# hebench/reference-seal-backend

Hardware: AMD Instinct MI355X
Metric: ciphertext-ops/sec (CKKS ct x ct mul+relin+rescale, N=2^15, L=16) (higher is better)
Workload: dtype u64 (exact residues; fp64-FMA engine for primes < 2^47, u64 Harvey engine with the fold reduction for the 60-bit primes)

## Files before the change

### reference-seal-backend_amd/csrc/he355_api.hip

```cpp
#include <hip/hip_runtime.h>

#include <array>
#include <algorithm>
#include <cerrno>
#include <cstdlib>
#include <cstdio>
#include <cstring>
#include <map>
#include <random>
#include <memory>
#include <stdexcept>
#include <string>
#include <vector>

#include "../../include/he355.h"
#include "device_pool.h"
#include "he355_internal.h"
#include "he355_kernels.h"
#include "he_params.h"
#include "ntt_core.h"
#include "client/he_client.h"
#include "client/multiword.h"

namespace he355 {
// ... 630 lines not shown
                const K1Mode mode = product ? K1_MUL : galois ? K1_GALOIS : K1_CT3;
                launch_k1(env, L, mode, nc, off, src.a, src.b, src.ix, src.table, B, src.addend, in_k3 && product, in_k3 && !product,
                          grouped ? &groups : nullptr, in_k3 && galois);
                key_switch_tail(env, L, nc, S, shape, in_k3 && product ? relin_scaled() : src.key, ops, grouped ? &groups : nullptr, off, ro, fork);
                return;
            }
            if (fork) HIPCHECK(hipEventRecord(fork, env.stream));
        });
        HIPCHECK(hipGetLastError());
        return groups.sum_out != nullptr;
    }
    void key_switch_tail(const KernelEnv &env, int L, u64 nc, const Scratch &S, KsShape shape, const u64 *key, const K3Fuse &ops,
                         const KsGroups *groups, u64 g_off, u64 *rescale_out, hipEvent_t fork)
    {
        const KsBuffers &B = S.ks;
        const size_t N = P.N, LN = (size_t)L * N;
        const int SP = (int)P.K - 1;
        const bool lat = shape == KsShape::Latency;
        launch_k2(env, L, nc, B, nullptr, 0, lat ? kLatTargets : 1);
        if (fork) HIPCHECK(hipEventRecord(fork, env.stream));
        if (lat) {
            u64 *part = latency_partials((size_t)std::max(kLatSplit, kLatSplitU64) * nc * 2 * (L + 1) * N, env.stream == stream2_ ? 1 : 0);
            launch_k3(env, L, nc, B, key, K3_ALL, nullptr, kLatSplit, part, kLatSplitU64);
            launch_k3_combine(env, L, nc, B, kLatSplit, part, kLatSplitU64);
            launch_floor_cols(env, SP, L, nc * 2, B.tpr, B.e, 0, 0, nullptr, 0, kLatTargets);
        } else if (shape == KsShape::Unfused) {
            launch_k3(env, L, nc, B, key, K3_ALL, nullptr, 1, nullptr, 0, groups, g_off);
            launch_floor_cols(env, SP, L, nc * 2, B.tpr, B.e);
        } else {
            launch_k3(env, L, nc, B, key, K3_SPECIAL_ONLY, nullptr, 1, nullptr, 0, groups, g_off);
            K3Fuse f = ops;
            f.cols = B.e; f.c01 = B.c01; f.c01_item_stride = B.c01_item_stride; f.cols2 = nullptr; f.out = nullptr;
            if (rescale_out) {
                launch_floor_cols(env, SP, 1, nc * 2, B.tpr, B.e,  L - 1,  L);
                f.tt_lo = L - 1; f.tt_hi = L;
                launch_k3(env, L, nc, B, key, K3_DATA_ONLY, &f);
                launch_rows_inv_select(env, L - 1, nc * 2, B.c01 + (size_t)(L - 1) * N, (u64)LN, S.rlr);
                launch_floor_cols(env, L - 1, L - 1, nc * 2, S.rlr, S.f, 0, L - 1,  B.tpr, SP);
                f.tt_lo = 0; f.tt_hi = L - 1; f.cols2 = S.f; f.out = rescale_out;
                launch_k3(env, L, nc, B, key, K3_DATA_ONLY, &f);
                return;
            }
            launch_floor_cols(env, SP, L, nc * 2, B.tpr, B.e);
            f.tt_lo = 0; f.tt_hi = L;
            launch_k3(env, L, nc, B, key, K3_DATA_ONLY, &f, 1, nullptr, 0, groups, g_off);
            return;
        }
        FloorRowsArgs fr;
        fr.src_prime = SP; fr.n_tgt = L; fr.n_src = 2;
        fr.cols = B.e;
        fr.tsrc = B.t; fr.tsrc_op_stride = 2 * LN; fr.tsrc_poly_stride = LN;
        fr.addend = B.c01; fr.add_op_stride = B.c01_item_stride; fr.add_poly_stride = LN;
        fr.out = B.c01; fr.out_op_stride = B.c01_item_stride; fr.out_poly_stride = LN;
        fr.tail_prime = rescale_out ? L - 1 : -1;
        fr.tail = S.rlr;
        launch_floor_rows(env, nc, fr);
        if (rescale_out) rescale_tail(env, L, 2, nc, S, B.c01, 2 * LN, rescale_out);
    }
    void rescale_tail(const KernelEnv &env, int L, int size, u64 nc, const Scratch &S, const u64 *src, u64 src_op_stride, u64 *out)
    {
        const size_t N = P.N, LN = (size_t)L * N, L1N = (size_t)(L - 1) * N;
        launch_floor_cols(env, L - 1, L - 1, nc * size, S.rlr, S.f, 0, 0, nullptr, 0, latency_shape(env, nc) ? kLatTargets : 1);
        FloorRowsArgs fr;
        fr.src_prime = L - 1; fr.n_tgt = L - 1; fr.n_src = size;
        fr.cols = S.f;
        fr.tsrc = src; fr.tsrc_op_stride = src_op_stride; fr.tsrc_poly_stride = LN;
        fr.addend = nullptr; fr.add_op_stride = 0; fr.add_poly_stride = 0;
        fr.out = out; fr.out_op_stride = (u64)size * L1N; fr.out_poly_stride = L1N;
        fr.tail_prime = -1; fr.tail = nullptr;
        launch_floor_rows(env, nc, fr);
    }
// ... 1570 lines not shown
```

### reference-seal-backend_amd/csrc/he355_kernels.h

```cpp
#pragma once
#include <hip/hip_runtime.h>

#include <cstdlib>
#include <utility>

#include "device_types.h"
#include "behz_core.h"
#include "bfv_level_core.h"
#include "bfv_noise_core.h"

namespace he355 {

struct FloorConst {
    u64 inv, inv_shoup;
    double inv_d, inv_i;
    u64 half_mod;
    u64 src_mod;
};

struct KernelProbe {
    static constexpr int kCap = 2048;
    hipEvent_t start[kCap], stop[kCap];
    int created = 0, used = 0;
    u64 ops = 0;
// ... 13 lines not shown



struct KsBuffers {
    u64 *c01;
    u64 c01_item_stride;
    u64 *c2n;
    u64 *c2r;
    u64 *d;
    u64 *t;
    u64 *tp;
    u64 *tpr;
    u64 *e;
};
struct KsGroups {
    const uint32_t *const *perm = nullptr;
    const u64 *const *key = nullptr;
    const u32 *src_block = nullptr;
    u32 group_size = 0;
    u64 *sum_out = nullptr;
    const u32 *count = nullptr;
};
constexpr u32 kGroupKeepBit = 0x80000000u;
constexpr int kMoveListCap = 64;
enum K1Mode { K1_MUL = 0, K1_CT3 = 1, K1_GALOIS = 2 };
enum K3Part { K3_ALL = 0, K3_SPECIAL_ONLY = 1, K3_DATA_ONLY = 2 };
struct K3Fuse {
    const u64 *cols;
    u64 *c01;
    u64 c01_item_stride;
    int tt_lo, tt_hi;
    const u64 *cols2;
    u64 *out;
    const u64 *ta = nullptr, *tb = nullptr;
    Indexer tix{};
    u64 t_op_offset = 0;
    int c1_mode = 0;
    const u64 *c1_src = nullptr;
    const u64 *gsrc = nullptr;
    const uint32_t *gperm = nullptr;
    u64 gsrc_op_offset = 0;
};
inline bool k3_can_fuse(const KernelEnv &env) { return env.scheme == 2 && env.K >= 2; }
struct FloorRowsArgs {
    int src_prime, n_tgt, n_src;
    const u64 *cols;
    const u64 *tsrc; u64 tsrc_op_stride, tsrc_poly_stride;
    const u64 *addend; u64 add_op_stride, add_poly_stride;
    u64 *out; u64 out_op_stride, out_poly_stride;
    int tail_prime;
    u64 *tail;
};


struct CrtTablesDev {
    int L, words;
    const u64 *Q, *halfQ, *punct, *inv;
    double Qd;
    u64 t;
};

struct EncTablesDev {
    const uint32_t *slot_index;
    const void *W, *Z;
};

// ... 93 lines not shown
```

### reference-seal-backend_amd/csrc/he355_kernels.hip

```cpp
#include <hip/hip_runtime.h>

#include <cstdio>
#include <cstdlib>
#include <stdexcept>
#include <type_traits>

#include "he355_kernels.h"
#include "ntt_core.h"
#include "client/ckks_codec.h"
#include "client/multiword.h"
#include "client/sampler.h"

#if !defined(HE355_KNS) || !defined(HE355_U64_FOLD)
#error "he355_kernels.hip is compiled once per form of the u64 engine: -DHE355_KNS=ks_shoup -DHE355_U64_FOLD=0 and -DHE355_KNS=ks_fold -DHE355_U64_FOLD=1 (Makefile)"
#endif
namespace he355 {
namespace HE355_KNS {
namespace {

#include "kernel_common.inc"

template <class Ar>
__device__ __forceinline__ void rows_fwd_job(const PrimeDev &P, u64 *row, bool in_raw, u32 rowbase, int lane, u64 *lds, bool valid)
{
// ... 952 lines not shown
        if (valid) store_rowC(A.t + (ok * A.L + tt) * N + rowoff, lane, v);
        return;
    }
    const bool last = A.logn1 == 0;
    u64 *dst = tt < A.L ? A.t + (ok * A.L + tt) * N + rowoff : A.tpr + ok * N + rowoff;
    if (P.f64) {
        const ArF64 ar = make_ar(P, (ArF64 *)nullptr);
        double x[kRowE];
#pragma unroll
        for (int r = 0; r < kRowE; ++r) x[r] = ar.from_canon(v[r]);
        wave_rows_inv(ar, P, last, n1 + a_row, lane, lds[wave], x);
#pragma unroll
        for (int r = 0; r < kRowE; ++r) v[r] = last ? ar.to_canon(x[r]) : ar.to_raw(x[r]);
    } else {
        const ArU64 ar = make_ar(P, (ArU64 *)nullptr);
        u64 x[kRowE];
#pragma unroll
        for (int r = 0; r < kRowE; ++r) x[r] = v[r];
        wave_rows_inv(ar, P, last, n1 + a_row, lane, lds[wave], x);
#pragma unroll
        for (int r = 0; r < kRowE; ++r) v[r] = last ? ar.to_canon(x[r]) : ar.to_raw(x[r]);
    }
    if (valid) store_rowA(dst, lane, v);
}

struct FloorColsArgs {
    const u64 *src;
    u64 *dst;
    int src_prime, n_tgt, K;
    const FloorConst *fc;
    int tgt_first, dst_ntgt;
    const u64 *src2;
    int src2_prime;
    u64 f64_mask;
    int tsplit;
};

template <int LOGN1>
__device__ __forceinline__ void floor_source_column(const PrimeDev &Ps, const u64 *src, int col, u64 c[1 << LOGN1])
{
    constexpr int N1 = 1 << LOGN1;
    if (LOGN1 == 0) {
        c[0] = src[col];
    } else if (Ps.f64) {
        const ArF64 ar = make_ar(Ps, (ArF64 *)nullptr);
        double x[N1];
#pragma unroll
        for (int a = 0; a < N1; ++a) x[a] = ar.from_raw(src[(a << kRowLog) + col]);
        col_inv<ArF64, LOGN1>(ar, x, ctw(Ps.inv), Ps.inv_w0_scaled);
#pragma unroll
        for (int a = 0; a < N1; ++a) c[a] = ar.to_canon(x[a]);
    } else {
        const ArU64 ar = make_ar(Ps, (ArU64 *)nullptr);
        u64 x[N1];
#pragma unroll
        for (int a = 0; a < N1; ++a) x[a] = src[(a << kRowLog) + col];
        col_inv<ArU64, LOGN1>(ar, x, ctw(Ps.inv), Ps.inv_w0_scaled);
#pragma unroll
        for (int a = 0; a < N1; ++a) c[a] = ar.to_canon(x[a]);
    }
    const u64 qs = Ps.q, half = qs >> 1;
#pragma unroll
    for (int a = 0; a < N1; ++a) c[a] = addmod(c[a], half, qs);
}

struct FcnConsts {
    double half1, half2;
    double inv2, inv2_i;
    double pow32, qd, qinv;
    double recentre;
};

template <int LOGN1, bool MERGE, bool WIDE1>
__device__ __forceinline__ void fcn_targets_f64(const FloorColsArgs &A, const PrimeDev *primes, u64 poly, int col, u64 mask,
                                                const typename std::conditional<WIDE1, u64, double>::type (&c)[1 << LOGN1],
                                                const u64 *park , bool wide2, const FcnConsts *ctab)
{
    constexpr int N1 = 1 << LOGN1;
    constexpr u64 N = (u64)N1 << kRowLog;
    constexpr int LA = LOGN1 < 4 ? LOGN1 : 4;
    if (!mask) return;
    const u32 off8 = (u32)col << 3;
// ... 60 lines not shown
        store_word_rows<N1>(poly_rsrc(A.dst + (poly * A.dst_ntgt + t) * N, (u32)N1 * kSlotBytes), off8, v);
        if (!m) break;
        t = tn; wa = wa_n; k = kn;
    }
}

template <int LOGN1, bool MERGE>
__global__ void __launch_bounds__(kBlock, 2) k_floor_colsn(FloorColsArgs A, const PrimeDev *primes)
{
    constexpr int N1 = 1 << LOGN1;
    constexpr u64 N = (u64)N1 << kRowLog;
    const u64 poly = blockIdx.x >> 2;
    const int col = ((blockIdx.x & 3) << 8) | threadIdx.x;
    __shared__ u64 park[MERGE ? N1 : 1][MERGE ? kBlock : 1];
    __shared__ FcnConsts ctab[kMaxPrimes];
    const PrimeDev &Ps = primes[A.src_prime];
    const u64 qs = Ps.q, qs2 = MERGE ? primes[A.src2_prime].q : 0;
    if ((int)threadIdx.x >= A.tgt_first && (int)threadIdx.x < A.tgt_first + A.n_tgt) {
        const int i = threadIdx.x;
        const PrimeDev &Pi = primes[i];
        FcnConsts k;
        k.half1 = (double)A.fc[A.src_prime * A.K + i].half_mod;
        k.half2 = 0; k.inv2 = 0; k.inv2_i = 0;
        int flags = qs > 2 * Pi.q ? 1 : 0;
        if (MERGE) {
            const FloorConst f2 = A.fc[A.src2_prime * A.K + i];
            k.half2 = (double)f2.half_mod; k.inv2 = f2.inv_d; k.inv2_i = f2.inv_i;
            flags |= qs2 > 2 * Pi.q ? 2 : 0;
        }
        k.pow32 = Pi.pow32; k.qd = Pi.qd; k.qinv = Pi.qinv; k.recentre = (double)flags;
        ctab[i] = k;
    }
    u64 c[N1];
    floor_source_column<LOGN1>(Ps, A.src + poly * N, col, c);
    if constexpr (MERGE) {
        u64 c2[N1];
        floor_source_column<LOGN1>(primes[A.src2_prime], A.src2 + poly * N, col, c2);
#pragma unroll
        for (int a = 0; a < N1; ++a) park[a][threadIdx.x] = c2[a];
    }
    __syncthreads();
    u64 tgt = ((A.tgt_first + A.n_tgt >= 64 ? ~(u64)0 : (((u64)1 << (A.tgt_first + A.n_tgt)) - 1))) & ~(((u64)1 << A.tgt_first) - 1);
    tgt = split_mask(tgt, (int)blockIdx.y, A.tsplit);
    const u64 f64t = tgt & A.f64_mask;
    const bool wide2 = MERGE && (qs2 >> 52) != 0;
    if (qs >> 52) {
        fcn_targets_f64<LOGN1, MERGE, true>(A, primes, poly, col, f64t, c, &park[0][0], wide2, ctab);
    } else {
        double cd[N1];
#pragma unroll
        for (int a = 0; a < N1; ++a) cd[a] = u52_to_f64(c[a]);
        fcn_targets_f64<LOGN1, MERGE, false>(A, primes, poly, col, f64t, cd, &park[0][0], wide2, ctab);
#pragma unroll
        for (int a = 0; a < N1; ++a) c[a] = f64_to_u52(cd[a]);
    }
    const u32 off8 = (u32)col << 3;
    for (u64 m = tgt & ~A.f64_mask; m; m &= m - 1) {
        const int i = __builtin_ctzll(m);
        const PrimeDev &Pi = primes[i];
        const u64 qi = Pi.q;
        const u64 half_i = A.fc[A.src_prime * A.K + i].half_mod;
        const ModU64 mi = make_modu(Pi);
        const ArU64 ar = make_ar(Pi, (ArU64 *)nullptr);
        u64 dl[N1];
#pragma unroll
        for (int a = 0; a < N1; ++a) dl[a] = submod(qs > qi ? barrett64(c[a], mi) : c[a], half_i, qi);
        if constexpr (MERGE) {
            const FloorConst f2 = A.fc[A.src2_prime * A.K + i];
#pragma unroll
            for (int a = 0; a < N1; ++a) {
                const u64 v2 = park[a][threadIdx.x];
                const u64 d1 = submod(qs2 > qi ? barrett64(v2, mi) : v2, f2.half_mod, qi);
// ... 721 lines not shown
    case L1:                                                                                                                  \
        if (wide) hipLaunchKernelGGL((k_k2n<L1, true>), gd, dim3(kBlock), 0, env.stream, AK[wide], env.primes);               \
        else hipLaunchKernelGGL((k_k2n<L1, false>), gd, dim3(kBlock), 0, env.stream, AK[wide], env.primes);                   \
        break;
        switch (env.logn1) { HE355_K2N(0) HE355_K2N(1) HE355_K2N(2) HE355_K2N(3) HE355_K2N(4) HE355_K2N(5) }
#undef HE355_K2N
    }
}


void launch_k3(const KernelEnv &env, int L, u64 n_ops, const KsBuffers &buf, const u64 *key, K3Part part, const K3Fuse *fuse, int n_split, u64 *split_part,
               int n_split_u64, const KsGroups *groups, u64 g_op_offset)
{
    if (groups && (n_split > 1 || (fuse && fuse->ta))) throw std::runtime_error("grouped keys: the 8-wave rotation instantiations only");
    if (n_split_u64 <= 0) n_split_u64 = n_split;
    if (n_split > 1 && (fuse || !split_part)) throw std::runtime_error("digit-split K3: unfused launches with a partial-sum buffer only");
    const unsigned char *prime_f64 = env.prime_f64;
    if (!n_ops) return;
    if (fuse && (part != K3_DATA_ONLY || !k3_can_fuse(env))) throw std::runtime_error("fused mod-down: data-prime tiles only");
    struct { K3Args A; unsigned g; bool f64; int waves; } pend[2];
    int n_pend = 0;
    for (int pass = 0; pass < 2; ++pass) {
        K3Args A;
        A.d = buf.d; A.c2n = buf.c2n; A.key = key; A.t = buf.t; A.tp = buf.tp; A.tpr = buf.tpr;
        A.n_ops = n_ops; A.L = L; A.K = env.K; A.logn1 = env.logn1; A.ckks = env.scheme == 2;
        A.cols = fuse ? fuse->cols : nullptr; A.c01 = fuse ? fuse->c01 : nullptr; A.c01_item_stride = fuse ? fuse->c01_item_stride : 0;
        A.cols2 = fuse ? fuse->cols2 : nullptr; A.out2 = fuse ? fuse->out : nullptr;
        A.c1_mode = fuse ? fuse->c1_mode : 0; A.c1_src = fuse ? fuse->c1_src : nullptr;
        A.gsrc = fuse ? fuse->gsrc : nullptr; A.gperm = fuse ? fuse->gperm : nullptr; A.gsrc_op_offset = fuse ? fuse->gsrc_op_offset : 0;
        if ((A.c1_mode == 4 || A.c1_mode == 5) && (!A.gsrc || (!groups && !A.gperm))) throw std::runtime_error("gathered rotation: the input slab and its permutation are needed");
        if (A.c1_mode == 5 && !A.c1_src) throw std::runtime_error("gathered rotation with addend: the addend rows are needed");
        A.ta = fuse ? fuse->ta : nullptr; A.tb = fuse ? fuse->tb : nullptr; A.tix = fuse ? fuse->tix : Indexer{}; A.t_op_offset = fuse ? fuse->t_op_offset : 0;
        if (fuse && fuse->cols2 && fuse->tt_hi > L - 1) throw std::runtime_error("fused rescale: only primes below the one divided out");
        A.fc = env.floor_consts;
        A.n_split = n_split > 1 ? (pass == 0 ? n_split : n_split_u64) : 1; A.part = split_part;
        A.n_tt = 0;
        A.n_q = 0;
        for (int t = 0; t < env.K; ++t) A.n_q += prime_f64[t] == 0;
        A.keyq_offset = (u64)env.Ltop * 2 * env.K * env.N;
        A.keyq = key ? key + A.keyq_offset : nullptr;
        A.groups = groups ? *groups : KsGroups{}; A.g_op_offset = g_op_offset;
        for (int tt = 0; tt <= L; ++tt) {
            if ((part == K3_SPECIAL_ONLY && tt != L) || (part == K3_DATA_ONLY && tt == L)) continue;
            if (fuse && (tt < fuse->tt_lo || tt >= fuse->tt_hi)) continue;
            const int t = (tt == L) ? env.K - 1 : tt;
            if ((prime_f64[t] != 0) == (pass == 0)) {
                int slot = 0;
                for (int u = 0; u < t; ++u) slot += prime_f64[u] == 0;
                A.q_slot[A.n_tt] = (unsigned char)slot;
                A.tt_list[A.n_tt++] = (unsigned char)tt;
            }
        }
        if (!A.n_tt) continue;
        int waves = A.n_split > 1 ? 1 : 8;
        const u64 tiles = (u64)A.n_tt << env.logn1;
        u64 n_og = 0;
        u32 ogpb = 1;
        unsigned g = 0;
        auto size_grid = [&](int w) {
            n_og = (n_ops + w - 1) / w;
            const u32 og_max = w == 8 ? (n_og >= 128 ? 4 : 2) : 4;
            ogpb = og_max;
            {
                const double work = (pass == 0 ? 7.0 : 14.0) * (L + 2) * (w == 4 ? 0.5 : 1.0), startup = 4.0;
                double best = 0;
                for (u32 c = og_max; c >= 1; c >>= 1) {
                    const u64 blocks = tiles * ((n_og + c - 1) / c);
                    const double cost = (double)((blocks + 255) / 256) * (c * work + startup);
                    if (c == og_max || cost < best * 0.999) { best = cost; ogpb = c; }
                }
            }
            const u64 n_ogb = (n_og + ogpb - 1) / ogpb;
            g = (unsigned)(((tiles + 7) / 8) * 8 * n_ogb);
        };
        size_grid(waves);
        const bool level_sum = groups && groups->sum_out && fuse;
        if (level_sum) {
            const u64 gs8 = groups->group_size / 8;
            if (waves != 8 || groups->group_size % 8 || n_ops % groups->group_size || g_op_offset % groups->group_size)
                throw std::runtime_error("level sum in k_k3: fused 8-wave launches over whole groups of a multiple of eight ciphertexts");
            ogpb = (u32)(n_og / gs8);
            g = (unsigned)(((tiles + 7) / 8) * 8 * gs8);
        }
        if (pass == 1 && waves == 8 && g <= 128 && !level_sum) {
            size_grid(4);
            if (g + (n_pend ? pend[0].g : 0) <= 256) waves = 4;
            else size_grid(8);
        }
        A.og_per_block = ogpb;
        A.og_stride = level_sum ? (u32)(groups->group_size / 8) : 1u;
        pend[n_pend].A = A; pend[n_pend].g = g; pend[n_pend].f64 = pass == 0; pend[n_pend].waves = waves;
        ++n_pend;
    }
    const hipStream_t st3 = env.stream;
    const bool tensor = fuse && fuse->ta;
    if (n_pend == 2 && pend[0].waves == 1) {
        const unsigned ny = (unsigned)std::max(pend[0].A.n_split, pend[1].A.n_split);
        hipLaunchKernelGGL(k_k3_dual, dim3(pend[0].g + pend[1].g, ny), dim3(64), 0, st3, pend[0].A, pend[1].A, pend[1].g, env.primes);
        return;
    }
    if (n_pend == 2 && pend[0].waves == 8 && pend[0].g + pend[1].g <= kDualMaxBlocksK3) {
        const dim3 gd(pend[0].g + pend[1].g);
#define HE355_K3D8(F, T, G)                                                                                                                     \
    do {                                                                                                                                        \
        if (pend[1].waves == 4) hipLaunchKernelGGL((k_k3_dual8<F, T, G, 4>), gd, dim3(512), 0, st3, pend[0].A, pend[1].A, pend[1].g, env.primes); \
        else hipLaunchKernelGGL((k_k3_dual8<F, T, G, 8>), gd, dim3(512), 0, st3, pend[0].A, pend[1].A, pend[1].g, env.primes);                    \
    } while (0)
        if (groups) { if (fuse) HE355_K3D8(true, false, true); else HE355_K3D8(false, false, true); }
        else if (tensor) HE355_K3D8(true, true, false);
        else if (fuse) HE355_K3D8(true, false, false);
        else HE355_K3D8(false, false, false);
#undef HE355_K3D8
        return;
    }
    for (int i = 0; i < n_pend; ++i) {
        const K3Args &A = pend[i].A;
        const unsigned g = pend[i].g;
        const bool f64 = pend[i].f64;
        KernelProbe *pr = f64 && pend[i].waves == 8 ? env.probe : nullptr;
        int slot = -1;
        if (pr && pr->used < KernelProbe::kCap) {
            slot = pr->used++;
            if (slot >= pr->created) {
                (void)hipEventCreate(&pr->start[slot]);
                (void)hipEventCreate(&pr->stop[slot]);
                pr->created = slot + 1;
            }
            pr->ops += n_ops;
            (void)hipEventRecord(pr->start[slot], env.stream);
        }
        if (pend[i].waves == 1) {
            const dim3 gd(g, (unsigned)A.n_split);
            if (f64) hipLaunchKernelGGL((k_k3<ArF64, 1>), gd, dim3(64), 0, st3, A, env.primes);
            else hipLaunchKernelGGL((k_k3<ArU64, 1>), gd, dim3(64), 0, st3, A, env.primes);
        } else if (pend[i].waves == 4) {
            if (groups && fuse) hipLaunchKernelGGL((k_k3<ArU64, 4, true, false, true>), dim3(g), dim3(256), 0, st3, A, env.primes);
            else if (groups) hipLaunchKernelGGL((k_k3<ArU64, 4, false, false, true>), dim3(g), dim3(256), 0, st3, A, env.primes);
            else if (tensor) hipLaunchKernelGGL((k_k3<ArU64, 4, true, true>), dim3(g), dim3(256), 0, st3, A, env.primes);
            else if (fuse) hipLaunchKernelGGL((k_k3<ArU64, 4, true>), dim3(g), dim3(256), 0, st3, A, env.primes);
            else hipLaunchKernelGGL((k_k3<ArU64, 4>), dim3(g), dim3(256), 0, st3, A, env.primes);
        } else if (groups) {
            if (f64 && fuse) hipLaunchKernelGGL((k_k3<ArF64, 8, true, false, true>), dim3(g), dim3(512), 0, st3, A, env.primes);
            else if (f64) hipLaunchKernelGGL((k_k3<ArF64, 8, false, false, true>), dim3(g), dim3(512), 0, st3, A, env.primes);
            else if (fuse) hipLaunchKernelGGL((k_k3<ArU64, 8, true, false, true>), dim3(g), dim3(512), 0, st3, A, env.primes);
            else hipLaunchKernelGGL((k_k3<ArU64, 8, false, false, true>), dim3(g), dim3(512), 0, st3, A, env.primes);
        } else if (f64) {
            if (tensor) hipLaunchKernelGGL((k_k3<ArF64, 8, true, true>), dim3(g), dim3(512), 0, st3, A, env.primes);
            else if (fuse) hipLaunchKernelGGL((k_k3<ArF64, 8, true>), dim3(g), dim3(512), 0, st3, A, env.primes);
            else hipLaunchKernelGGL((k_k3<ArF64, 8>), dim3(g), dim3(512), 0, st3, A, env.primes);
        } else {
            if (tensor) hipLaunchKernelGGL((k_k3<ArU64, 8, true, true>), dim3(g), dim3(512), 0, st3, A, env.primes);
            else if (fuse) hipLaunchKernelGGL((k_k3<ArU64, 8, true>), dim3(g), dim3(512), 0, st3, A, env.primes);
            else hipLaunchKernelGGL((k_k3<ArU64, 8>), dim3(g), dim3(512), 0, st3, A, env.primes);
        }
        if (slot >= 0) (void)hipEventRecord(pr->stop[slot], env.stream);
    }
}

void launch_k3_combine(const KernelEnv &env, int L, u64 n_ops, const KsBuffers &buf, int n_split, const u64 *split_part, int n_split_u64)
{
    if (n_split_u64 <= 0) n_split_u64 = n_split;
    if (!n_ops) return;
    K3CombineArgs A;
    A.part = split_part; A.t = buf.t; A.tpr = buf.tpr; A.n_ops = n_ops; A.n_split = n_split; A.n_split_u64 = n_split_u64; A.L = L; A.K = env.K; A.logn1 = env.logn1;
    A.ckks = env.scheme == 2;
    const u64 jobs = (n_ops * 2 * (u64)(L + 1)) << env.logn1;
    hipLaunchKernelGGL(k_k3_combine, dim3(grid_for(jobs, kWaves)), dim3(kBlock), 0, env.stream, A, env.primes);
}

void launch_floor_cols(const KernelEnv &env, int src_prime, int n_tgt, u64 n_polys, const u64 *src, u64 *dst, int tgt_first, int dst_ntgt, const u64 *src2,
                       int src2_prime, int tsplit)
{
    if (!n_polys || n_tgt <= 0) return;
    FloorColsArgs A;
    A.src = src; A.dst = dst; A.src_prime = src_prime; A.n_tgt = n_tgt; A.K = env.K; A.fc = env.floor_consts;
    A.tgt_first = tgt_first; A.dst_ntgt = dst_ntgt > 0 ? dst_ntgt : n_tgt;
    A.src2 = src2; A.src2_prime = src2_prime;
    A.tsplit = tsplit > 1 ? tsplit : 1;
    const dim3 g((unsigned)(n_polys * 4), (unsigned)A.tsplit);
    A.f64_mask = 0;
    for (int t = 0; t < env.K; ++t) A.f64_mask |= (u64)(env.prime_f64[t] != 0) << t;
#define HE355_FCN(L1)                                                                                                          \
    case L1:                                                                                                                   \
        if (src2) hipLaunchKernelGGL((k_floor_colsn<L1, true>), g, dim3(kBlock), 0, env.stream, A, env.primes);                \
        else hipLaunchKernelGGL((k_floor_colsn<L1, false>), g, dim3(kBlock), 0, env.stream, A, env.primes);                    \
        break;
    switch (env.logn1) { HE355_FCN(0) HE355_FCN(1) HE355_FCN(2) HE355_FCN(3) HE355_FCN(4) HE355_FCN(5) }
#undef HE355_FCN
}

void launch_floor_rows(const KernelEnv &env, u64 n_ops, const FloorRowsArgs &args)
{
    const unsigned char *prime_f64 = env.prime_f64;
    if (!n_ops) return;
    const u64 n_jobs = n_ops * args.n_src;
    u32 jpb = 8 * kWaves;
    while (jpb > (u32)kWaves && (((u64)args.n_tgt << env.logn1) * ((n_jobs + jpb - 1) / jpb) < 256u * 8 || jpb / 2 >= n_jobs)) jpb >>= 1;
    if (args.tail_prime < 0) {
        FloorRowsDev AE[2];
        unsigned ge[2] = {0, 0};
        for (int e = 0; e < 2; ++e) {
            FloorRowsDev &A = AE[e];
            A.a = args; A.fc = env.floor_consts; A.n_ops = n_ops; A.K = env.K; A.logn1 = env.logn1;
            A.jobs_per_block = jpb;
            A.n_i = 0;
            for (int i = 0; i < args.n_tgt; ++i)
                if ((prime_f64[i] != 0) == (e == 0)) A.i_list[A.n_i++] = (unsigned char)i;
            ge[e] = (unsigned)((((u64)A.n_i) << env.logn1) * ((n_jobs + jpb - 1) / jpb));
        }
        if (ge[0] && ge[1] && (n_ops <= 8 || ge[0] + ge[1] <= kDualMaxBlocks)) {
// ... 222 lines not shown
```

### reference-seal-backend_amd/csrc/he355_launchers.inc

```
void launch_ntt_forward(const KernelEnv &env, const PolyView &v, u32 n_items);
void launch_ntt_inverse(const KernelEnv &env, const PolyView &v, u32 n_items);
void launch_addsub(const KernelEnv &env, int L, int size, u64 n_results, const u64 *a, const u64 *b, Indexer ix, u64 *out, bool sub);
void launch_mul3(const KernelEnv &env, int L, u64 n_results, const u64 *a, const u64 *b, Indexer ix, u64 *out);
void launch_plain_op(const KernelEnv &env, int L, int size, u64 n_results, const u64 *ct, const u64 *pt, Indexer ix, u64 *out, int mode);
void launch_drop_residues(const KernelEnv &env, int L, int L_to, u64 n_polys, const u64 *in, u64 *out);
void launch_sum_cts(const KernelEnv &env, int L, int size, u64 n_terms, const u64 *in, u64 *out, u64 n_out = 1, bool accumulate = false);
void launch_mul3_acc(const KernelEnv &env, int L, u64 rows, u64 cols, int inner, const u64 *a, u64 a_stride_i, u64 a_stride_k, const u64 *b,
                     u64 b_stride_k, u64 b_stride_j, u64 *out);
void launch_sum_groups(const KernelEnv &env, int L, u64 n_cts, u32 n_groups, const u64 *in, const u32 *d_mult, u64 *out);
void launch_move_cts(const KernelEnv &env, u64 *dst, const u64 *src, const uint32_t *idx, u64 n, u64 elems_per_ct, bool scatter);
void launch_k1(const KernelEnv &env, int L, K1Mode mode, u64 n_ops, u64 op_offset, const u64 *a, const u64 *b, Indexer ix,
               const uint32_t *perm, const KsBuffers &buf, const u64 *addend = nullptr, bool no_c01 = false, bool no_c1 = false,
               const KsGroups *groups = nullptr, bool no_c0n = false);
void launch_k2(const KernelEnv &env, int L, u64 n_ops, const KsBuffers &buf, const u64 *src = nullptr, u64 src_op_stride = 0, int tsplit = 1);
void launch_k3(const KernelEnv &env, int L, u64 n_ops, const KsBuffers &buf, const u64 *key, K3Part part = K3_ALL, const K3Fuse *fuse = nullptr,
               int n_split = 1, u64 *split_part = nullptr, int n_split_u64 = 0,
               const KsGroups *groups = nullptr, u64 g_op_offset = 0);
void launch_k3_combine(const KernelEnv &env, int L, u64 n_ops, const KsBuffers &buf, int n_split, const u64 *split_part, int n_split_u64 = 0);
void launch_floor_cols(const KernelEnv &env, int src_prime, int n_tgt, u64 n_polys, const u64 *src, u64 *dst, int tgt_first = 0, int dst_ntgt = 0,
                       const u64 *src2 = nullptr, int src2_prime = 0, int tsplit = 1);
void launch_floor_rows(const KernelEnv &env, u64 n_ops, const FloorRowsArgs &args);
void launch_behz_extend(const KernelEnv &env, const BehzDev &bz, const BehzSrc &src, u64 n_cts, u64 *xq, u64 *xbsk);
bool behz_cols_fusable(const KernelEnv &env, const BehzDev &bz);
void launch_behz_extend_cols(const KernelEnv &env, const BehzDev &bz, const BehzSrc &src, u64 n_cts, u64 *xq, u64 *xbsk);
void launch_behz_tensor_inv(const KernelEnv &env, const BehzDev &bz, const BehzSrc &src, u64 n_ops, u64 op_offset, const u64 *eq, const u64 *ebsk, u64 *dq,
                            u64 *ds);
void launch_rows_fwd(const KernelEnv &env, const PolyView &v, u32 n_items);
void launch_behz_cols_floor_sk(const KernelEnv &env, const BehzDev &bz, u64 n_ops, const u64 *dq, const u64 *ds, u64 *out);
void launch_behz_rows_tensor(const KernelEnv &env, const BehzDev &bz, u64 n_ops, const u64 *xq, const u64 *xbsk, u64 *dq, u64 *ds);
void launch_cols_fwd(const KernelEnv &env, const PolyView &v, u32 n_items);
void launch_cols_inv(const KernelEnv &env, const PolyView &v, u32 n_items);
void launch_behz_floor_sk(const KernelEnv &env, const BehzDev &bz, u64 n_ops, const u64 *dq, const u64 *ds, u64 *out);
void launch_bfv_galois(const KernelEnv &env, int L, u64 n_ops, const u64 *in, const uint32_t *gather, u64 *c01, u64 c01_item_stride, u64 *tgt,
                       const u64 *addend = nullptr);
void launch_bfv_tail_sp(const KernelEnv &env, u64 n_polys, const u64 *tpr, u64 *rp);
void launch_bfv_tail_fin(const KernelEnv &env, int L, u64 n_ops, const u64 *t, const u64 *rp, u64 *c01, u64 c01_item_stride, const u64 *add01 = nullptr,
                         u64 add01_item_stride = 0);
void launch_rows_inv_select(const KernelEnv &env, int prime, u64 n_polys, const u64 *src, u64 src_poly_stride, u64 *tail);
void launch_enc_sample(const KernelEnv &env, u64 n_cts, u64 seed, u64 first_index, u64 *u, u64 *e);
void launch_enc_mul_pk(const KernelEnv &env, u64 n_cts, const u64 *u, const u64 *pk, u64 *z, bool add_in);
void launch_divround_last_coeff(const KernelEnv &env, u64 n_polys, const u64 *z, u64 *out);
void launch_dot_sk(const KernelEnv &env, int L, int size, u64 n_cts, const u64 *ct, const u64 *sk, u64 *out);
void launch_bfv_scale_round(const KernelEnv &env, u64 n_cts, const u64 *phase, u64 *plain, const CrtTablesDev &c);
void launch_ckks_encode(const KernelEnv &env, u64 n_vec, const double *values, u64 count, double scale, void *zbuf, u64 *plain, const EncTablesDev &t, int *err);
void launch_ckks_decode(const KernelEnv &env, u64 n_vec, const u64 *coeff, double scale, void *zbuf, double *out, const EncTablesDev &t, const CrtTablesDev &c,
                        const SlotRanges &sr);
void launch_bfv_encode_scatter(const KernelEnv &env, u64 n_vec, const long long *values, u64 count, u64 *ev, const uint32_t *slot_index, u64 t);
void launch_bfv_decode_gather(const KernelEnv &env, u64 n_vec, const u64 *ev, long long *out, const uint32_t *slot_index, u64 t, const SlotRanges &sr);
void launch_keygen_kswitch(const KernelEnv &env, u64 *key, u64 *e_scratch, u64 *target_scratch, const u64 *sk, const uint32_t *perm, u64 seed, u64 key_id);
bool ks_lds_supported(const KernelEnv &env, int L);
u64 ks_lds_part_words(const KernelEnv &env, int L);
void launch_ks_lds(const KernelEnv &env, int L, u64 n_ops, const LdsKsOperands &src, const u64 *key, u64 *part, u64 *out, u64 out_op_stride);
void launch_rescale_lds(const KernelEnv &env, int L, int size, u64 n_ops, const u64 *src, u64 src_op_stride, u64 *out);
// ... 11 lines not shown
```

### reference-seal-backend_amd/csrc/k3_body.inc

```
    static_assert(!TENSOR || FUSE, "the operand rows enter through the fused epilogue's sums");
    static_assert(!GROUPED || !TENSOR, "grouped keys are for rotations");
    constexpr int kWaves = WAVES, kBlock = WAVES * 64;
    typedef typename Ar::T T;
    typedef typename Ar::Acc Acc;
    constexpr bool kF64 = std::is_same<Ar, ArF64>::value;
    constexpr bool kPacked = kF64;
    constexpr int kDigitPieces = kPacked ? 6 : 8;
    K3_LDS_DECL
    const int wave = threadIdx.x >> 6, lane = threadIdx.x & 63;
    const u32 n1 = 1u << A.logn1;
    const u64 N = (u64)n1 << kRowLog;
    const u64 n_og = (A.n_ops + kWaves - 1) / kWaves;
    const u64 n_ogb = (n_og + A.og_per_block - 1) / A.og_per_block;
    const u64 total_tiles = (u64)A.n_tt * n1;
    const u64 s = K3_BID_X >> 3, xcd = K3_BID_X & 7;
    const u64 tile = (s / n_ogb) * 8 + xcd;
    if (tile >= total_tiles) return;
    const u64 og_first = A.og_stride > 1 ? s % n_ogb : (s % n_ogb) * A.og_per_block;
    const int tt = A.tt_list[tile >> A.logn1];
    const int q_slot = A.q_slot[tile >> A.logn1];
    const u32 a_row = (u32)(tile & (n1 - 1));
    const int t = (tt == A.L) ? A.K - 1 : tt;
    const PrimeDev &P = primes[t];
    const Ar ar = make_ar(P, (Ar *)nullptr);
    const u64 rowoff = (u64)a_row << kRowLog;
    const auto twr = stage_row_twiddles<Ar, kBlock>(P, ar, n1 + a_row, twl_raw);
    __syncthreads();
    for (u32 g = 0; g < A.og_per_block; ++g) {
        const u64 og = og_first + (u64)g * A.og_stride;
        if (og >= n_og) break;
        u64 op = og * kWaves + wave;
        const bool valid = op < A.n_ops;
        if (!valid) op = A.n_ops - 1;
// ... 75 lines not shown
            const uint32_t *pm;
            const u64 *p0 = gather_base(poly, pm);
#pragma unroll
            for (int r = 0; r < kRowE; ++r) v[r] = p0[pm[elemC(lane, r)]];
        };
        const bool has_own = A.ckks && tt < A.L;
        const int nd = A.L - (has_own ? 1 : 0);
        auto digit = [&](int i) -> int { return (has_own && i >= tt) ? i + 1 : i; };
        const int split = FUSE ? 1 : (A.n_split > 1 ? A.n_split : 1), grp = split > 1 ? (int)K3_BID_Y : 0;
        const int i_begin = nd * grp / split, i_end = nd * (grp + 1) / split;
        auto src_row = [&](int j) -> const u64 * { return A.d + ((op * (A.L + 1) + tt) * A.L + j) * N + rowoff; };
        if (i_begin < i_end) dma_row_to_lds<kDigitPieces>(src_row(digit(i_begin)), stage[wave], lane);
        tensor_init();
        if (has_own && grp == 0) {
            if constexpr (TENSOR) {
                const u64 tr = A.t_op_offset + op;
                const u64 LNt = (u64)A.L * N;
                u64 a1[kRowE], b1[kRowE];
                load_rowC(A.ta + (idx_a(A.tix, tr) * 2 + 1) * LNt + (u64)tt * N + rowoff, lane, a1);
                load_rowC(A.tb + (idx_b(A.tix, tr) * 2 + 1) * LNt + (u64)tt * N + rowoff, lane, b1);
                T x[kRowE];
#pragma unroll
                for (int r = 0; r < kRowE; ++r) x[r] = ar.from_canon(ar.dy_out(ar.dy_mul(ar.dy_in(a1[r]), ar.dy_in(b1[r]))));
                mac_digit(x, tt);
            } else {
                T x[kRowE];
                u64 v[kRowE];
                load_rowC(FUSE && A.c1_mode == 3 ? A.c1_src + (op * 3 + 2) * ((u64)A.L * N) + (u64)tt * N + rowoff : A.c2n + (op * A.L + tt) * N + rowoff, lane, v);
#pragma unroll
                for (int r = 0; r < kRowE; ++r) x[r] = ar.from_canon(v[r]);
                mac_digit(x, tt);
            }
        }
        if constexpr (FUSE) {
            const bool resc = A.cols2 != nullptr;
            const int n_rows = nd + 2;
            const u64 LN = (u64)A.L * N, L1N = (u64)(A.L - 1) * N;
            auto row_ptr = [&](int i) -> const u64 * {
                if (i < nd) return src_row(digit(i));
                if (!resc) return A.cols + ((op * 2 + (i - nd)) * A.L + tt) * N + rowoff;
                return A.cols2 + ((op * 2 + (i - nd)) * (A.L - 1) + tt) * N + rowoff;
            };
            const FloorConst fc = A.fc[(A.K - 1) * A.K + t];
            const FloorConst fc2 = A.fc[(resc ? A.L - 1 : 0) * A.K + t];
            if (nd == 0) dma_row_to_lds(row_ptr(0), stage[wave], lane);
            for (int i = 0; i < nd; ++i) {
                T x[1][kRowE];
                asm volatile("s_waitcnt vmcnt(0)" ::: "memory");
                if constexpr (kPacked) {
                    lds_rowA48(stage[wave], lane, x[0]);
                } else {
                    u64 v[kRowE];
                    lds_rowA(stage[wave], lane, v);
#pragma unroll
                    for (int r = 0; r < kRowE; ++r) x[0][r] = ar.from_raw(v[r]);
                }
                asm volatile("s_waitcnt lgkmcnt(0)" ::: "memory");
                if (i + 1 < nd) dma_row_to_lds<kDigitPieces>(row_ptr(i + 1), stage[wave], lane);
                else dma_row_to_lds(row_ptr(i + 1), stage[wave], lane);
                if constexpr (!Ar::kKeyQuotient) {
                    u64 kv0[kRowE], kv1[kRowE];
                    const int j = digit(i);
                    wave_rows_fwd_n(ar, twr, lane, lds[wave], x, [&]() { load_rowC(key_row(j, 0), lane, kv0); load_rowC(key_row(j, 1), lane, kv1); });
                    if constexpr (kF64) {
#pragma unroll
                        for (int r0 = 0; r0 < kRowE; r0 += kMacG / 2) {
                            double xs[kMacG], ks[kMacG], pr[kMacG];
#pragma unroll
                            for (int k = 0; k < kMacG / 2; ++k) {
                                xs[2 * k] = x[0][r0 + k]; ks[2 * k] = ar.key_in(kv0[r0 + k]);
                                xs[2 * k + 1] = x[0][r0 + k]; ks[2 * k + 1] = ar.key_in(kv1[r0 + k]);
                            }
                            ar.template mulmod_vv_g<kMacG>(xs, ks, pr);
#pragma unroll
                            for (int k = 0; k < kMacG / 2; ++k) { acc0[r0 + k] += pr[2 * k]; acc1[r0 + k] += pr[2 * k + 1]; }
                        }
                    }
                } else {
                    wave_rows_fwd_n<Ar, decltype(twr), NoHook, true>(ar, twr, lane, lds[wave], x);
                    mac_digit(x[0], digit(i));
                }
            }
            acc_flush();
#pragma unroll 1
            for (int i = nd; i < n_rows; ++i) {
                T x[1][kRowE];
                u64 v[kRowE], av[kRowE];
                asm volatile("s_waitcnt vmcnt(0)" ::: "memory");
                lds_rowA(stage[wave], lane, v);
#pragma unroll
                for (int r = 0; r < kRowE; ++r) x[0][r] = ar.from_raw(v[r]);
                asm volatile("s_waitcnt lgkmcnt(0)" ::: "memory");
                if (i + 1 < n_rows) dma_row_to_lds(row_ptr(i + 1), stage[wave], lane);
                const int k = i - nd;
                u64 *c01_row = A.c01 + op * A.c01_item_stride + k * LN + (u64)tt * N + rowoff;
                if constexpr (TENSOR) {
                } else if (k == 0 && A.c1_mode == 4) {
                    gather_row(0, av);
                } else if (k == 0 && A.c1_mode == 5) {
                    u64 ad[kRowE];
                    load_rowC(A.c1_src + (op * 2 + 0) * LN + (u64)tt * N + rowoff, lane, ad);
                    gather_row(0, av);
#pragma unroll
                    for (int r = 0; r < kRowE; ++r) av[r] = addmod(av[r], ad[r], P.q);
                } else if (k == 1 && (A.c1_mode == 1 || A.c1_mode == 4)) {
#pragma unroll
                    for (int r = 0; r < kRowE; ++r) av[r] = 0;
                } else if (A.c1_mode == 3) {
                    load_rowC(A.c1_src + (op * 3 + k) * LN + (u64)tt * N + rowoff, lane, av);
                } else {
                    load_rowC(k == 1 && (A.c1_mode == 2 || A.c1_mode == 5) ? A.c1_src + (op * 2 + 1) * LN + (u64)tt * N + rowoff : c01_row, lane, av);
                }
                bool into_sum = false;
                u64 *sum_row = nullptr;
                u32 sum_cnt = 0;
                if constexpr (GROUPED && !TENSOR) {
                    if (A.groups.sum_out) {
                        const u32 gop = (u32)(A.g_op_offset + op), gi = __builtin_amdgcn_readfirstlane(gop / A.groups.group_size);
// ... 21 lines not shown
#pragma unroll
                        for (int r = 0; r < kRowE; ++r) v[r] = ar.floor_fin_s(ar.acc_canon(acc[r]), x[0][r], fc.inv, fc.inv_shoup, fc.inv_d, fc.inv_i);
                        if (valid) store_rowC(c01_row, lane, v);
                    } else {
#pragma unroll
                        for (int r = 0; r < kRowE; ++r) v[r] = ar.floor_fin2_s(ar.acc_canon(acc[r]), x[0][r], fc2);
                        if (valid) store_rowC(A.out2 + (op * 2 + k) * L1N + (u64)tt * N + rowoff, lane, v);
                    }
                } else if (!resc) {
#pragma unroll
                    for (int r = 0; r < kRowE; ++r) v[r] = ar.floor_fin(ar.acc_canon(acc[r]), x[0][r], fc.inv, fc.inv_shoup, fc.inv_d, fc.inv_i, av[r]);
                    if constexpr (GROUPED) {
                        if (into_sum) {
                            if (valid) store_rowC(sum_row, lane, v);
                        } else if (A.groups.sum_out) {
                            if (valid && (sum_cnt & kGroupKeepBit)) store_rowC(c01_row, lane, v);
                            const u32 m = sum_cnt & ~kGroupKeepBit;
                            if (m) {
                                u64 o[kRowE];
                                load_rowC(sum_row, lane, o);
                                for (u32 rep = 0; rep < m; ++rep)
#pragma unroll
                                    for (int r = 0; r < kRowE; ++r) o[r] = addmod(o[r], v[r], P.q);
                                if (valid) store_rowC(sum_row, lane, o);
                            }
                        } else if (valid) store_rowC(c01_row, lane, v);
                    } else if (valid) store_rowC(c01_row, lane, v);
                } else {
#pragma unroll
                    for (int r = 0; r < kRowE; ++r) v[r] = ar.floor_fin2(ar.acc_canon(acc[r]), x[0][r], fc, fc2, av[r]);
                    if (valid) store_rowC(A.out2 + (op * 2 + k) * L1N + (u64)tt * N + rowoff, lane, v);
                }
            }
        } else {
            for (int i = i_begin; i < i_end; ++i) {
                T x[1][kRowE];
                asm volatile("s_waitcnt vmcnt(0)" ::: "memory");
                if constexpr (kPacked) {
                    lds_rowA48(stage[wave], lane, x[0]);
                } else {
                    u64 v[kRowE];
                    lds_rowA(stage[wave], lane, v);
#pragma unroll
                    for (int r = 0; r < kRowE; ++r) x[0][r] = ar.from_raw(v[r]);
                }
                asm volatile("s_waitcnt lgkmcnt(0)" ::: "memory");
                if (i + 1 < i_end) dma_row_to_lds<kDigitPieces>(src_row(digit(i + 1)), stage[wave], lane);
                wave_rows_fwd_n<Ar, decltype(twr), NoHook, true>(ar, twr, lane, lds[wave], x);
                mac_digit(x[0], digit(i));
            }
            acc_flush();
            const bool inv_here = tt == A.L || !A.ckks;
            const bool last = A.logn1 == 0;
#pragma unroll 1
            for (int k = 0; k < 2; ++k) {
                u64 v[kRowE];
                const Acc *acc = k == 0 ? acc0 : acc1;
#pragma unroll
                for (int r = 0; r < kRowE; ++r) v[r] = ar.acc_canon(acc[r]);
                if (split > 1) {
                    if (valid) store_rowC(A.part + (((u64)grp * A.n_ops * 2 + op * 2 + k) * (A.L + 1) + tt) * N + rowoff, lane, v);
                    continue;
                }
                if (!inv_here) {
                    if (valid) store_rowC(A.t + ((op * 2 + k) * A.L + tt) * N + rowoff, lane, v);
                    continue;
                }
                T x[kRowE];
#pragma unroll
                for (int r = 0; r < kRowE; ++r) x[r] = ar.from_canon(v[r]);
                wave_rows_inv(ar, P, last, n1 + a_row, lane, lds[wave], x);
#pragma unroll
                for (int r = 0; r < kRowE; ++r) v[r] = last ? ar.to_canon(x[r]) : ar.to_raw(x[r]);
                u64 *dst = tt < A.L ? A.t + ((op * 2 + k) * A.L + tt) * N + rowoff : A.tpr + (op * 2 + k) * N + rowoff;
                if (valid) store_rowA(dst, lane, v);
            }
        }
    }
```

Baseline: 22400.

## Fuse last-prime tail of ct x ct rescale into k3 raw-tail variant

For the tensor (ct x ct) rescale path, the top data prime's row is now produced by a new k3 variant (TENSOR without FUSE). It does the inverse row transform directly into the rescale scratch buffer. This drops a separate floor_cols launch and a rows_inv_select launch. The following floor_cols pass subtracts the special-prime floor correction in its fp64 column pass (sub2) instead of relying on the earlier pass. The aim is fewer kernel launches and less global memory traffic per multiply, at the cost of a new kernel instantiation and more complex correction logic.

```diff
diff --git a/reference-seal-backend_amd/csrc/he355_api.hip b/reference-seal-backend_amd/csrc/he355_api.hip
--- a/reference-seal-backend_amd/csrc/he355_api.hip
+++ b/reference-seal-backend_amd/csrc/he355_api.hip
@@ -686,11 +686,18 @@
             K3Fuse f = ops;
             f.cols = B.e; f.c01 = B.c01; f.c01_item_stride = B.c01_item_stride; f.cols2 = nullptr; f.out = nullptr;
             if (rescale_out) {
-                launch_floor_cols(env, SP, 1, nc * 2, B.tpr, B.e,  L - 1,  L);
+                const bool raw = ops.ta != nullptr;
                 f.tt_lo = L - 1; f.tt_hi = L;
-                launch_k3(env, L, nc, B, key, K3_DATA_ONLY, &f);
-                launch_rows_inv_select(env, L - 1, nc * 2, B.c01 + (size_t)(L - 1) * N, (u64)LN, S.rlr);
-                launch_floor_cols(env, L - 1, L - 1, nc * 2, S.rlr, S.f, 0, L - 1,  B.tpr, SP);
+                if (raw) {
+                    f.raw_tail = S.rlr;
+                    launch_k3(env, L, nc, B, key, K3_DATA_ONLY, &f);
+                    f.raw_tail = nullptr;
+                } else {
+                    launch_floor_cols(env, SP, 1, nc * 2, B.tpr, B.e,  L - 1,  L);
+                    launch_k3(env, L, nc, B, key, K3_DATA_ONLY, &f);
+                    launch_rows_inv_select(env, L - 1, nc * 2, B.c01 + (size_t)(L - 1) * N, (u64)LN, S.rlr);
+                }
+                launch_floor_cols(env, L - 1, L - 1, nc * 2, S.rlr, S.f, 0, L - 1,  B.tpr, SP, 1,  raw);
                 f.tt_lo = 0; f.tt_hi = L - 1; f.cols2 = S.f; f.out = rescale_out;
                 launch_k3(env, L, nc, B, key, K3_DATA_ONLY, &f);
                 return;
diff --git a/reference-seal-backend_amd/csrc/he355_kernels.h b/reference-seal-backend_amd/csrc/he355_kernels.h
--- a/reference-seal-backend_amd/csrc/he355_kernels.h
+++ b/reference-seal-backend_amd/csrc/he355_kernels.h
@@ -69,6 +69,7 @@
     int tt_lo, tt_hi;
     const u64 *cols2;
     u64 *out;
+    u64 *raw_tail = nullptr;
     const u64 *ta = nullptr, *tb = nullptr;
     Indexer tix{};
     u64 t_op_offset = 0;
diff --git a/reference-seal-backend_amd/csrc/he355_kernels.hip b/reference-seal-backend_amd/csrc/he355_kernels.hip
--- a/reference-seal-backend_amd/csrc/he355_kernels.hip
+++ b/reference-seal-backend_amd/csrc/he355_kernels.hip
@@ -1008,22 +1008,30 @@
     int tgt_first, dst_ntgt;
     const u64 *src2;
     int src2_prime;
+    int sub2;
     u64 f64_mask;
     int tsplit;
 };
 
-template <int LOGN1>
-__device__ __forceinline__ void floor_source_column(const PrimeDev &Ps, const u64 *src, int col, u64 c[1 << LOGN1])
+template <int LOGN1, bool SUB = false>
+__device__ __forceinline__ void floor_source_column(const PrimeDev &Ps, const u64 *src, int col, u64 c[1 << LOGN1], const double *sub = nullptr)
 {
     constexpr int N1 = 1 << LOGN1;
+    static_assert(!SUB || LOGN1 > 0, "the correction rides the fp64 column pass");
     if (LOGN1 == 0) {
         c[0] = src[col];
-    } else if (Ps.f64) {
+    } else if (SUB || Ps.f64) {
         const ArF64 ar = make_ar(Ps, (ArF64 *)nullptr);
         double x[N1];
 #pragma unroll
         for (int a = 0; a < N1; ++a) x[a] = ar.from_raw(src[(a << kRowLog) + col]);
         col_inv<ArF64, LOGN1>(ar, x, ctw(Ps.inv), Ps.inv_w0_scaled);
+        if constexpr (SUB) {
+            const double half = u52_to_f64(Ps.q >> 1);
+#pragma unroll
+            for (int a = 0; a < N1; ++a) c[a] = ar.to_canon(x[a] - sub[a] + half);
+            return;
+        }
 #pragma unroll
         for (int a = 0; a < N1; ++a) c[a] = ar.to_canon(x[a]);
     } else {
@@ -1150,12 +1158,39 @@
         ctab[i] = k;
     }
     u64 c[N1];
-    floor_source_column<LOGN1>(Ps, A.src + poly * N, col, c);
     if constexpr (MERGE) {
         u64 c2[N1];
         floor_source_column<LOGN1>(primes[A.src2_prime], A.src2 + poly * N, col, c2);
 #pragma unroll
         for (int a = 0; a < N1; ++a) park[a][threadIdx.x] = c2[a];
+        if (A.sub2) {
+            const FloorConst fs = A.fc[A.src2_prime * A.K + A.src_prime];
+            bool done = false;
+            if constexpr (LOGN1 > 0) {
+                if (Ps.f64) {
+                    const ArF64 ar = make_ar(Ps, (ArF64 *)nullptr);
+                    const double pow32 = Ps.pow32, half2 = (double)fs.half_mod;
+                    double d[N1];
+#pragma unroll
+                    for (int a = 0; a < N1; ++a) d[a] = ar.mulmod_c(lift_wide(ar, c2[a], pow32) - half2, fs.inv_d, fs.inv_i);
+                    floor_source_column<LOGN1, true>(Ps, A.src + poly * N, col, c, d);
+                    done = true;
+                }
+            }
+            if (!done) {
+                floor_source_column<LOGN1>(Ps, A.src + poly * N, col, c);
+                const ModU64 ms = make_modu(Ps);
+#pragma unroll
+                for (int a = 0; a < N1; ++a) {
+                    const u64 d1 = submod(qs2 > qs ? barrett64(c2[a], ms) : c2[a], fs.half_mod, qs);
+                    c[a] = submod(c[a], mulmod(d1, fs.inv, ms), qs);
+                }
+            }
+        } else {
+            floor_source_column<LOGN1>(Ps, A.src + poly * N, col, c);
+        }
+    } else {
+        floor_source_column<LOGN1>(Ps, A.src + poly * N, col, c);
     }
     __syncthreads();
     u64 tgt = ((A.tgt_first + A.n_tgt >= 64 ? ~(u64)0 : (((u64)1 << (A.tgt_first + A.n_tgt)) - 1))) & ~(((u64)1 << A.tgt_first) - 1);
@@ -1943,6 +1978,10 @@
         if (A.c1_mode == 5 && !A.c1_src) throw std::runtime_error("gathered rotation with addend: the addend rows are needed");
         A.ta = fuse ? fuse->ta : nullptr; A.tb = fuse ? fuse->tb : nullptr; A.tix = fuse ? fuse->tix : Indexer{}; A.t_op_offset = fuse ? fuse->t_op_offset : 0;
         if (fuse && fuse->cols2 && fuse->tt_hi > L - 1) throw std::runtime_error("fused rescale: only primes below the one divided out");
+        if (fuse && fuse->raw_tail) {
+            if (!fuse->ta || fuse->tt_hi != fuse->tt_lo + 1 || groups) throw std::runtime_error("raw tail: one prime of a ct x ct multiply");
+            A.tpr = fuse->raw_tail;
+        }
         A.fc = env.floor_consts;
         A.n_split = n_split > 1 ? (pass == 0 ? n_split : n_split_u64) : 1; A.part = split_part;
         A.n_tt = 0;
@@ -2004,7 +2043,7 @@
         ++n_pend;
     }
     const hipStream_t st3 = env.stream;
-    const bool tensor = fuse && fuse->ta;
+    const bool tensor = fuse && fuse->ta, raw_tail = fuse && fuse->raw_tail;
     if (n_pend == 2 && pend[0].waves == 1) {
         const unsigned ny = (unsigned)std::max(pend[0].A.n_split, pend[1].A.n_split);
         hipLaunchKernelGGL(k_k3_dual, dim3(pend[0].g + pend[1].g, ny), dim3(64), 0, st3, pend[0].A, pend[1].A, pend[1].g, env.primes);
@@ -2047,6 +2086,7 @@
         } else if (pend[i].waves == 4) {
             if (groups && fuse) hipLaunchKernelGGL((k_k3<ArU64, 4, true, false, true>), dim3(g), dim3(256), 0, st3, A, env.primes);
             else if (groups) hipLaunchKernelGGL((k_k3<ArU64, 4, false, false, true>), dim3(g), dim3(256), 0, st3, A, env.primes);
+            else if (raw_tail) hipLaunchKernelGGL((k_k3<ArU64, 4, false, true>), dim3(g), dim3(256), 0, st3, A, env.primes);
             else if (tensor) hipLaunchKernelGGL((k_k3<ArU64, 4, true, true>), dim3(g), dim3(256), 0, st3, A, env.primes);
             else if (fuse) hipLaunchKernelGGL((k_k3<ArU64, 4, true>), dim3(g), dim3(256), 0, st3, A, env.primes);
             else hipLaunchKernelGGL((k_k3<ArU64, 4>), dim3(g), dim3(256), 0, st3, A, env.primes);
@@ -2056,11 +2096,13 @@
             else if (fuse) hipLaunchKernelGGL((k_k3<ArU64, 8, true, false, true>), dim3(g), dim3(512), 0, st3, A, env.primes);
             else hipLaunchKernelGGL((k_k3<ArU64, 8, false, false, true>), dim3(g), dim3(512), 0, st3, A, env.primes);
         } else if (f64) {
-            if (tensor) hipLaunchKernelGGL((k_k3<ArF64, 8, true, true>), dim3(g), dim3(512), 0, st3, A, env.primes);
+            if (raw_tail) hipLaunchKernelGGL((k_k3<ArF64, 8, false, true>), dim3(g), dim3(512), 0, st3, A, env.primes);
+            else if (tensor) hipLaunchKernelGGL((k_k3<ArF64, 8, true, true>), dim3(g), dim3(512), 0, st3, A, env.primes);
             else if (fuse) hipLaunchKernelGGL((k_k3<ArF64, 8, true>), dim3(g), dim3(512), 0, st3, A, env.primes);
             else hipLaunchKernelGGL((k_k3<ArF64, 8>), dim3(g), dim3(512), 0, st3, A, env.primes);
         } else {
-            if (tensor) hipLaunchKernelGGL((k_k3<ArU64, 8, true, true>), dim3(g), dim3(512), 0, st3, A, env.primes);
+            if (raw_tail) hipLaunchKernelGGL((k_k3<ArU64, 8, false, true>), dim3(g), dim3(512), 0, st3, A, env.primes);
+            else if (tensor) hipLaunchKernelGGL((k_k3<ArU64, 8, true, true>), dim3(g), dim3(512), 0, st3, A, env.primes);
             else if (fuse) hipLaunchKernelGGL((k_k3<ArU64, 8, true>), dim3(g), dim3(512), 0, st3, A, env.primes);
             else hipLaunchKernelGGL((k_k3<ArU64, 8>), dim3(g), dim3(512), 0, st3, A, env.primes);
         }
@@ -2080,13 +2122,14 @@
 }
 
 void launch_floor_cols(const KernelEnv &env, int src_prime, int n_tgt, u64 n_polys, const u64 *src, u64 *dst, int tgt_first, int dst_ntgt, const u64 *src2,
-                       int src2_prime, int tsplit)
-{
+                       int src2_prime, int tsplit, bool sub2)
+{
+    if (sub2 && !src2) throw std::runtime_error("floor column pass: the earlier correction comes from the merged source");
     if (!n_polys || n_tgt <= 0) return;
     FloorColsArgs A;
     A.src = src; A.dst = dst; A.src_prime = src_prime; A.n_tgt = n_tgt; A.K = env.K; A.fc = env.floor_consts;
     A.tgt_first = tgt_first; A.dst_ntgt = dst_ntgt > 0 ? dst_ntgt : n_tgt;
-    A.src2 = src2; A.src2_prime = src2_prime;
+    A.src2 = src2; A.src2_prime = src2_prime; A.sub2 = sub2;
     A.tsplit = tsplit > 1 ? tsplit : 1;
     const dim3 g((unsigned)(n_polys * 4), (unsigned)A.tsplit);
     A.f64_mask = 0;
diff --git a/reference-seal-backend_amd/csrc/he355_launchers.inc b/reference-seal-backend_amd/csrc/he355_launchers.inc
--- a/reference-seal-backend_amd/csrc/he355_launchers.inc
+++ b/reference-seal-backend_amd/csrc/he355_launchers.inc
@@ -18,7 +18,7 @@
                const KsGroups *groups = nullptr, u64 g_op_offset = 0);
 void launch_k3_combine(const KernelEnv &env, int L, u64 n_ops, const KsBuffers &buf, int n_split, const u64 *split_part, int n_split_u64 = 0);
 void launch_floor_cols(const KernelEnv &env, int src_prime, int n_tgt, u64 n_polys, const u64 *src, u64 *dst, int tgt_first = 0, int dst_ntgt = 0,
-                       const u64 *src2 = nullptr, int src2_prime = 0, int tsplit = 1);
+                       const u64 *src2 = nullptr, int src2_prime = 0, int tsplit = 1, bool sub2 = false);
 void launch_floor_rows(const KernelEnv &env, u64 n_ops, const FloorRowsArgs &args);
 void launch_behz_extend(const KernelEnv &env, const BehzDev &bz, const BehzSrc &src, u64 n_cts, u64 *xq, u64 *xbsk);
 bool behz_cols_fusable(const KernelEnv &env, const BehzDev &bz);
diff --git a/reference-seal-backend_amd/csrc/k3_body.inc b/reference-seal-backend_amd/csrc/k3_body.inc
--- a/reference-seal-backend_amd/csrc/k3_body.inc
+++ b/reference-seal-backend_amd/csrc/k3_body.inc
@@ -1,4 +1,3 @@
-    static_assert(!TENSOR || FUSE, "the operand rows enter through the fused epilogue's sums");
     static_assert(!GROUPED || !TENSOR, "grouped keys are for rotations");
     constexpr int kWaves = WAVES, kBlock = WAVES * 64;
     typedef typename Ar::T T;
@@ -140,7 +139,7 @@
                 mac_digit(x, tt);
             }
         }
-        if constexpr (FUSE) {
+        if constexpr (FUSE || TENSOR) {
             const bool resc = A.cols2 != nullptr;
             const int n_rows = nd + 2;
             const u64 LN = (u64)A.L * N, L1N = (u64)(A.L - 1) * N;
@@ -151,7 +150,7 @@
             };
             const FloorConst fc = A.fc[(A.K - 1) * A.K + t];
             const FloorConst fc2 = A.fc[(resc ? A.L - 1 : 0) * A.K + t];
-            if (nd == 0) dma_row_to_lds(row_ptr(0), stage[wave], lane);
+            if (FUSE && nd == 0) dma_row_to_lds(row_ptr(0), stage[wave], lane);
             for (int i = 0; i < nd; ++i) {
                 T x[1][kRowE];
                 asm volatile("s_waitcnt vmcnt(0)" ::: "memory");
@@ -165,7 +164,7 @@
                 }
                 asm volatile("s_waitcnt lgkmcnt(0)" ::: "memory");
                 if (i + 1 < nd) dma_row_to_lds<kDigitPieces>(row_ptr(i + 1), stage[wave], lane);
-                else dma_row_to_lds(row_ptr(i + 1), stage[wave], lane);
+                else if constexpr (FUSE) dma_row_to_lds(row_ptr(i + 1), stage[wave], lane);
                 if constexpr (!Ar::kKeyQuotient) {
                     u64 kv0[kRowE], kv1[kRowE];
                     const int j = digit(i);
@@ -191,7 +190,7 @@
             }
             acc_flush();
 #pragma unroll 1
-            for (int i = nd; i < n_rows; ++i) {
+            for (int i = nd; FUSE && i < n_rows; ++i) {
                 T x[1][kRowE];
                 u64 v[kRowE], av[kRowE];
                 asm volatile("s_waitcnt vmcnt(0)" ::: "memory");
@@ -279,8 +278,9 @@
                     if (valid) store_rowC(A.out2 + (op * 2 + k) * L1N + (u64)tt * N + rowoff, lane, v);
                 }
             }
-        } else {
-            for (int i = i_begin; i < i_end; ++i) {
+        }
+        if constexpr (!FUSE) {
+            for (int i = i_begin; !TENSOR && i < i_end; ++i) {
                 T x[1][kRowE];
                 asm volatile("s_waitcnt vmcnt(0)" ::: "memory");
                 if constexpr (kPacked) {
@@ -297,14 +297,28 @@
                 mac_digit(x[0], digit(i));
             }
             acc_flush();
-            const bool inv_here = tt == A.L || !A.ckks;
+            const bool inv_here = TENSOR || tt == A.L || !A.ckks;
             const bool last = A.logn1 == 0;
+            if constexpr (TENSOR) {
+#pragma unroll
+                for (int r = 0; r < kRowE; ++r) stage[wave][(r << 6) | lane] = ar.acc_canon(acc1[r]);
+            }
 #pragma unroll 1
             for (int k = 0; k < 2; ++k) {
                 u64 v[kRowE];
-                const Acc *acc = k == 0 ? acc0 : acc1;
-#pragma unroll
-                for (int r = 0; r < kRowE; ++r) v[r] = ar.acc_canon(acc[r]);
+                if constexpr (TENSOR) {
+                    if (k == 0) {
+#pragma unroll
+                        for (int r = 0; r < kRowE; ++r) v[r] = ar.acc_canon(acc0[r]);
+                    } else {
+#pragma unroll
+                        for (int r = 0; r < kRowE; ++r) v[r] = stage[wave][(r << 6) | lane];
+                    }
+                } else {
+                    const Acc *acc = k == 0 ? acc0 : acc1;
+#pragma unroll
+                    for (int r = 0; r < kRowE; ++r) v[r] = ar.acc_canon(acc[r]);
+                }
                 if (split > 1) {
                     if (valid) store_rowC(A.part + (((u64)grp * A.n_ops * 2 + op * 2 + k) * (A.L + 1) + tt) * N + rowoff, lane, v);
                     continue;
@@ -319,7 +333,7 @@
                 wave_rows_inv(ar, P, last, n1 + a_row, lane, lds[wave], x);
 #pragma unroll
                 for (int r = 0; r < kRowE; ++r) v[r] = last ? ar.to_canon(x[r]) : ar.to_raw(x[r]);
-                u64 *dst = tt < A.L ? A.t + ((op * 2 + k) * A.L + tt) * N + rowoff : A.tpr + (op * 2 + k) * N + rowoff;
+                u64 *dst = tt < A.L && !TENSOR ? A.t + ((op * 2 + k) * A.L + tt) * N + rowoff : A.tpr + (op * 2 + k) * N + rowoff;
                 if (valid) store_rowA(dst, lane, v);
             }
         }
```

After: 22680, median of 6. 1.01x the previous value.
